# charleschen003/doudizhu-rl

Hardware: NVIDIA B200
Metric: env-steps/sec (legal moves + state encode) (higher is better)
Workload: dtype u64

## Files before the change

doudizhu-rl_b200/csrc/ddz_kernels.cu:

```cuda
#include <cuda.h>
#include <cuda_runtime.h>
#include <cstdint>
#include <cstdio>
#include <cstdlib>
#include <cstring>
#include <atomic>
#include <mutex>

#include "../../include/ddz_b200.h"
#include "ddz_device.cuh"
#include <cuda_bf16.h>
#include <math_constants.h>
#include "ddz_flat.cuh"
#include "ddz_search.cuh"

namespace ddz {

#ifndef DDZ_THREADS
#define DDZ_THREADS 64
#endif
constexpr int kThreads = DDZ_THREADS;
constexpr int kWarpsPerCta = kThreads / 32;
constexpr int kEnvs = 128;
constexpr int kWin = 320;
constexpr int kMinCtasPerSm = 28 / kWarpsPerCta;
#ifdef DDZ_PLAIN_STORES
#define DDZ_STORE(p, v) (*(p) = (v))
#else
#define DDZ_STORE(p, v) __stcs((p), (v))
#endif
#ifndef DDZ_HEAVY
#define DDZ_HEAVY 32
#endif
#ifndef DDZ_ROW_UNROLL
#define DDZ_ROW_UNROLL 4
#endif
#ifndef DDZ_LOOKBACK
#define DDZ_LOOKBACK 4
#endif
#ifndef DDZ_TILE_ENVS
#define DDZ_TILE_ENVS 32
#endif
constexpr int kTile = DDZ_TILE_ENVS;
constexpr int kRowUnroll = DDZ_ROW_UNROLL;
constexpr int kHeavy = DDZ_HEAVY;
#ifndef DDZ_PHASE_ORDER
#define DDZ_PHASE_ORDER 0
#endif
DDZ_DEV bool kFaceSecond(int t) { return DDZ_PHASE_ORDER == 0 ? (t & 1) != 0 : DDZ_PHASE_ORDER == 2; }
constexpr int kLookBack = DDZ_LOOKBACK;

enum Mode { kStepOnly = 0, kObserve = 1, kStepObserve = 2 };

#ifdef DDZ_PROB_FORM_B
constexpr int kProbForm = 1, kLutEntries = 16;
constexpr uint64_t kProbMark = 0x0008888888888888ull;
#else
constexpr int kProbForm = 0, kLutEntries = 8;
constexpr uint64_t kProbMark = 0ull;
#endif
DDZ_DEV float4 lut_entry(int i) {
    const int c = i & 7;
    return (i & 8) ? make_float4(c > 3 ? 1.f : 0.f, c > 2 ? 1.f : 0.f, c > 1 ? 1.f : 0.f, c > 0 ? 1.f : 0.f)
                   : make_float4(c > 0 ? 1.f : 0.f, c > 1 ? 1.f : 0.f, c > 2 ? 1.f : 0.f, c > 3 ? 1.f : 0.f);
}

struct WsHeader { unsigned int ticket, finished, epoch, auto_step; };
struct Workspace { WsHeader* h; unsigned long long* tile; };
static inline int ntiles(int B) { return (B + kTile - 1) / kTile; }
static inline int nblocks(int B) { return (B + kEnvs - 1) / kEnvs; }
static inline Workspace ws_of(void* p) {
    Workspace w; w.h = (WsHeader*)p; w.tile = (unsigned long long*)((char*)p + 256);
    return w;
}
constexpr unsigned long long kAggregate = 1ull << 32, kInclusive = 2ull << 32;

DDZ_DEV unsigned long long ld_relaxed(const unsigned long long* p) {
    unsigned long long v;
    asm volatile("ld.relaxed.gpu.global.u64 %0, [%1];" : "=l"(v) : "l"(p) : "memory");
    return v;
}
DDZ_DEV void st_relaxed(unsigned long long* p, unsigned long long v) {
    asm volatile("st.relaxed.gpu.global.u64 [%0], %1;" ::"l"(p), "l"(v) : "memory");
}

#ifdef DDZ_TRACE
__device__ unsigned long long* g_trace = nullptr;
DDZ_DEV void trace(int tile, int slot) {
    if (g_trace && (threadIdx.x & 31) == 0) {
        unsigned long long ts; asm volatile("mov.u64 %0, %globaltimer;" : "=l"(ts));
        g_trace[(size_t)tile * 8 + slot] = ts;
    }
}
#else
DDZ_DEV void trace(int, int) {}
#endif

DDZ_DEV long long warp_sum_ll(long long v) {
#pragma unroll
    for (int o = 16; o > 0; o >>= 1) v += __shfl_xor_sync(0xFFFFFFFFu, v, o);
    return v;
}
DDZ_DEV void stat_add(int64_t* stats, int slot, long long v) {
    const int s = __reduce_add_sync(0xFFFFFFFFu, (int)v);
    if ((threadIdx.x & 31) == 0 && s != 0 && stats) atomicAdd((unsigned long long*)&stats[slot], (unsigned long long)(long long)s);
}
DDZ_DEV void step_stats(int64_t* stats, unsigned int sf, const int32_t* rewards, int extra_err) {
    const int over = (sf >> 2) & 1, winner = (sf >> 3) & 3;
    stat_add(stats, 4, sf & 1);
    stat_add(stats, 9, (sf >> 1) & 1);
    stat_add(stats, 0, over);
    stat_add(stats, 1, over && winner == 1);
    stat_add(stats, 2, over && winner == 2);
    stat_add(stats, 3, over && winner == 0);
    stat_add(stats, 5, over ? (winner == 1 ? rewards[1] : -rewards[1]) : 0);
    stat_add(stats, 6, over ? (winner == 1 ? -(rewards[0] + rewards[2]) : rewards[0] + rewards[2]) : 0);
    stat_add(stats, 7, (int)((sf >> 5) & 3) + extra_err);
}


DDZ_DEV long long tile_lookback(const Workspace& ws, int t, unsigned long long epoch_tag, int total, int lane, int64_t* stats,
                                bool& timed_out) {
    constexpr unsigned FULL = 0xFFFFFFFFu;
    long long base = 0;
    timed_out = false;
    if (t <= 0) return 0;
    int p = t - 1;
    unsigned int spins = 0;
    bool finished = false;
    while (!finished) {
        unsigned long long w[kLookBack];
#pragma unroll
        for (int j = 0; j < kLookBack; j++) {
            const int idx = p - 32 * j - lane;
            w[j] = idx >= 0 ? ld_relaxed(&ws.tile[idx]) : (epoch_tag | kInclusive);
        }
#pragma unroll
        for (int j = 0; j < kLookBack; j++) {
            if (finished) break;
            const bool ok = ((w[j] >> 34) == (epoch_tag >> 34)) && ((w[j] >> 32) & 3ull) != 0;
            if (!__all_sync(FULL, ok)) {
                __nanosleep(64);
                if (++spins > (1u << 22)) {
                    if (lane == 0 && stats) atomicAdd((unsigned long long*)&stats[7], 1ull);
                    finished = true; timed_out = true;
                }
                break;
            }
            const unsigned int incmask = __ballot_sync(FULL, ((w[j] >> 32) & 3ull) == 2ull);
            const int stop = incmask ? (__ffs(incmask) - 1) : 31;
            base += warp_sum_ll(lane <= stop ? (long long)(unsigned int)w[j] : 0ll);
            p -= 32;
            if (incmask) finished = true;
        }
    }
    if (lane == 0) st_relaxed(&ws.tile[t], epoch_tag | kInclusive | (unsigned int)(base + total));
    return base;
}

__global__ void __launch_bounds__(kEnvs) k_reset(void* state, const int8_t* __restrict__ perm,
                                                 const int8_t* __restrict__ lord_pile, int pool_games,
                                                 int only_done, int64_t* stats, int B) {
    const int b = blockIdx.x * kEnvs + threadIdx.x, lane = threadIdx.x & 31;
    const bool valid = b < B;
    StateView v = view_of(state, B);
    Env e;
    if (valid) e = load_env(v, b); else e.meta = 0;
    const bool want = valid && (!only_done || e.done());
    const unsigned int need = __ballot_sync(0xFFFFFFFFu, want);
    const unsigned int bad = warp_deal(need, e, perm, lord_pile, pool_games, B, b, lane);
    if (want) store_env(v, b, e);
    if (lane == 0 && bad && stats) atomicAdd((unsigned long long*)&stats[7], (unsigned long long)__popc(bad));
}

struct RowLane {
    int first;
    int k;
    uint32_t sh;
    bool hi;
    DDZ_DEV static RowLane make(int lane) {
        RowLane r; r.first = lane / 15; r.k = lane - 15 * r.first; r.hi = r.k >= 8; r.sh = 4u * (uint32_t)(r.k & 7);
        if (lane >= 30) { r.first = 0x3FFFFFFF; r.k = 0; }
        return r;
    }
    DDZ_DEV const float4& thermo(uint64_t packed, const float4* lut) const {
        const uint32_t w = hi ? (uint32_t)(packed >> 32) : (uint32_t)packed;
        return lut[(w >> sh) & 15u];
    }
};
struct FaceRow { uint64_t packed; float s; float pad; };

template <class RowT>
DDZ_DEV void write_rows(float4* __restrict__ gdst, int nrows, const RowLane& rl, const float4* __restrict__ lut,
                        const RowT* __restrict__ rows);
template <>
DDZ_DEV void write_rows<FaceRow>(float4* __restrict__ gdst, int nrows, const RowLane& rl, const float4* __restrict__ lut,
                                 const FaceRow* __restrict__ rows) {
    float4* dst = gdst + (rl.first & 1) * 15 + rl.k;
#pragma unroll (kRowUnroll)
    for (int r = rl.first; r < nrows; r += 2, dst += 30) {
        const float4 raw = *reinterpret_cast<const float4*>(&rows[r]);
        const uint64_t packed = ((uint64_t)__float_as_uint(raw.y) << 32) | __float_as_uint(raw.x);
        const float s = raw.z;
        float4 q = rl.thermo(packed, lut);
        q.x *= s; q.y *= s; q.z *= s; q.w *= s;
        DDZ_STORE(dst, q);
    }
}
template <>
DDZ_DEV void write_rows<uint64_t>(float4* __restrict__ gdst, int nrows, const RowLane& rl, const float4* __restrict__ lut,
                                  const uint64_t* __restrict__ rows) {
    float4* dst = gdst + (rl.first & 1) * 15 + rl.k;
#pragma unroll (kRowUnroll)
    for (int r = rl.first; r < nrows; r += 2, dst += 30) DDZ_STORE(dst, rl.thermo(rows[r], lut));
}

template <int V> struct FaceCfg;
template <> struct FaceCfg<0> { static constexpr int C = 4; };
template <> struct FaceCfg<1> { static constexpr int C = 7; };
template <> struct FaceCfg<2> { static constexpr int C = 9; };
template <> struct FaceCfg<3> { static constexpr int C = 6; };

template <int V>
DDZ_DEV void face_planes(const Env& e, uint64_t* planes , float* p ) {
    int s = e.cur(), prev = (s + 2) % 3, next = (s + 1) % 3;
    uint64_t hand = pick3(s, e.hand[0], e.hand[1], e.hand[2]);
    uint64_t taken = e.hist[0] + e.hist[1] + e.hist[2];
    int n = 0;
    planes[n++] = hand;
    planes[n++] = taken;
    if (V == 1 || V == 2) {
        planes[n++] = pick3(prev, e.hist[0], e.hist[1], e.hist[2]);
        planes[n++] = pick3(s, e.hist[0], e.hist[1], e.hist[2]);
        planes[n++] = pick3(next, e.hist[0], e.hist[1], e.hist[2]);
    }
    if (V == 2 || V == 3) {
        planes[n++] = pick3(prev, e.recent[0], e.recent[1], e.recent[2]);
        planes[n++] = pick3(next, e.recent[0], e.recent[1], e.recent[2]);
    }
    uint64_t unknown = (kDeckPacked - taken - hand) | kProbMark;
    planes[n++] = unknown;
    planes[n++] = unknown;
    int size1 = card_count(pick3(next, e.hand[0], e.hand[1], e.hand[2]));
    int size2 = card_count(pick3(prev, e.hand[0], e.hand[1], e.hand[2]));
    int tot = size1 + size2;
    p[0] = tot > 0 ? __fdiv_rn((float)size1, (float)tot) : 0.f;
    p[1] = tot > 0 ? __fdiv_rn((float)size2, (float)tot) : 0.f;
}

struct StepArgs {
    const int32_t* offsets; const uint64_t* actions; const void* choice; int mode;
    uint64_t seed, env0; uint32_t stepno; int32_t rewards[3];
    const int8_t* perm; const int8_t* lord_pile; int pool_games;
    int8_t* r; uint8_t* done; int8_t* cat; float* reward;
    long long prev_cap;
};
struct OutArgs {
    int32_t* offsets; uint64_t* actions_u64; float4* actions_f32; long long cap; float4* face;
    int static_tiles;
};


struct SeqWindowEmitter {
    uint64_t* out; int pos, win;
    DDZ_DEV void operator()(uint64_t mv) { if ((unsigned)pos < (unsigned)win) out[pos] = mv; pos++; }
};
struct WindowEmitter {
    uint64_t* out; int base, win;
    DDZ_DEV void operator()(int idx, uint64_t mv) { const unsigned rel = (unsigned)(base + idx); if (rel < (unsigned)win) out[rel] = mv; }
};

struct __align__(128) WarpSmem {
    FaceRow face[32 * 9];
    uint64_t moves[kWin];
    float4 lut[kLutEntries];
};

template <int V, int MODE>
__global__ void __launch_bounds__(kThreads, kMinCtasPerSm) k_env(void* state, StepArgs a, OutArgs o,
                                                  Workspace ws, int64_t* stats, int B) {
    constexpr bool STEP = (MODE == kStepOnly || MODE == kStepObserve);
    constexpr bool EMIT = (MODE != kStepOnly);
    constexpr int C = FaceCfg<(V < 0 ? 0 : V)>::C;
    constexpr unsigned FULL = 0xFFFFFFFFu;
    extern __shared__ __align__(128) unsigned char smem_raw[];
    const int lane = threadIdx.x & 31, wib = threadIdx.x >> 5;
    WarpSmem& sm = reinterpret_cast<WarpSmem*>(smem_raw)[wib];
    const RowLane rl = RowLane::make(lane);
    const int nt = (B + kTile - 1) / kTile;
    const unsigned int nwarps = gridDim.x * kWarpsPerCta;

    int t = blockIdx.x * kWarpsPerCta + wib;
    unsigned int epoch = 0, autostep = 0, stepno = a.stepno;
    if (EMIT) {
        if (lane == 0) {
            if (!o.static_tiles) t = (int)atomicAdd(&ws.h->ticket, 1u);
            epoch = ws.h->epoch; autostep = ws.h->auto_step;
        }
        if (!o.static_tiles) t = __shfl_sync(FULL, t, 0);
        if (lane < kLutEntries) sm.lut[lane] = lut_entry(lane);
        __syncwarp();
    }
    if (t < nt) {
    const int b0 = t * kTile, b = b0 + lane;
    const bool valid = lane < kTile && b < B;
    const int nenv = min(kTile, B - b0);
    trace(t, 0);

    Env e;
    e.meta = 0;
    uint64_t hand = 0, last = 0;
    Masks hm{0, 0, 0, 0};
    Rule ru{true, 0, 1, 0};
    int n = 0;
    unsigned int sf = 0;
    int prev_off = 0, prev_end = 0;
    uint64_t choice_raw = 0;
    if (valid) {
        if (STEP) {
            prev_off = a.offsets[b]; prev_end = a.offsets[b + 1];
            if (a.mode == DDZ_CHOICE_MOVE) choice_raw = ((const uint64_t*)a.choice)[b];
            else if (a.mode != DDZ_CHOICE_PHILOX) choice_raw = ((const uint32_t*)a.choice)[b];
        }
        e = load_env(view_of(state, B), b);
        if (STEP && a.perm) {
            const char* prow = reinterpret_cast<const char*>(a.perm) +
                               54 * ((size_t)((e.meta >> 8) % (uint32_t)a.pool_games) * B + b);
            asm volatile("prefetch.global.L2 [%0];" ::"l"(prow));
            asm volatile("prefetch.global.L2 [%0];" ::"l"(prow + 53));
        }
    }
    if (EMIT) {
        epoch = __shfl_sync(FULL, epoch, 0);
        autostep = __shfl_sync(FULL, autostep, 0);
        if (STEP && a.stepno == DDZ_STEPNO_AUTO) stepno = autostep;
    }
    const unsigned long long epoch_tag = (unsigned long long)(epoch & 0x3FFFFFFFu) << 34;
    if (valid) {
        if (STEP) {
            int o_r = 0, o_cat = -1;
            float rw0 = 0.f, rw1 = 0.f, rw2 = 0.f;
            if (!e.done()) {
                const int base = prev_off, full = prev_end - prev_off;
                const int cnt = a.prev_cap >= 0 ? (int)max(0ll, min((long long)full, a.prev_cap - base)) : full;
                long long idx = -1;
                if (a.mode == DDZ_CHOICE_INDEX) idx = (int32_t)(uint32_t)choice_raw;
                else if (a.mode == DDZ_CHOICE_MOD) idx = cnt > 0 ? (long long)((uint32_t)choice_raw % (uint32_t)cnt) : -1;
                else if (a.mode == DDZ_CHOICE_PHILOX) idx = cnt > 0 ? (long long)(philox(a.seed, a.env0 + (uint64_t)b, stepno) % (uint32_t)cnt) : -1;
                else {
                    const uint64_t want = choice_raw;
                    for (int i = 0; i < cnt; i++) if (a.actions[base + i] == want) { idx = i; break; }
                }
                if (idx < 0 || idx >= cnt) {
                    sf += 32u;
                    if (!(cnt == 0 && full > 0)) e.meta |= 0x20u;
                } else {
                    const uint64_t mv = a.actions[base + idx];
                    StepOut so = apply_move(e, mv, a.rewards);
                    o_r = so.r; o_cat = so.cat; rw0 = so.reward[0]; rw1 = so.reward[1]; rw2 = so.reward[2];
                    sf |= 1u | (so.pass ? 2u : 0u);
                    if (so.done) sf |= 4u | ((unsigned int)so.winner << 3);
                }
            }
            if (a.r) a.r[b] = (int8_t)o_r;
            if (a.done) a.done[b] = (uint8_t)e.done();
            if (a.cat) a.cat[b] = (int8_t)o_cat;
            if (a.reward) { a.reward[3 * (size_t)b] = rw0; a.reward[3 * (size_t)b + 1] = rw1; a.reward[3 * (size_t)b + 2] = rw2; }
        }
    }
    {
        if (STEP) {
            if (a.perm) {
                const unsigned int need = __ballot_sync(FULL, valid && e.done());
                sf += ((warp_deal(need, e, a.perm, a.lord_pile, a.pool_games, B, b, lane) >> lane) & 1u) << 5;
            }
            if (valid) store_env(view_of(state, B), b, e);
        }
        if (valid && EMIT && !e.done()) {
            hand = hand_to_move(e); last = trick_of(e);
            hm = masks_of(hand); ru = rule_of(last); n = count_legal(hm, ru, last != 0);
        }
    }
    if (STEP && !EMIT) step_stats(stats, sf, a.rewards, 0);
    if (EMIT) {
    int inc = n;
#pragma unroll
    for (int d = 1; d < 32; d <<= 1) { int u = __shfl_up_sync(FULL, inc, d); if (lane >= d) inc += u; }
    const int local = inc - n;
    const int total = __shfl_sync(FULL, inc, 31);
    if (lane == 0) st_relaxed(&ws.tile[t], epoch_tag | (t == 0 ? kInclusive : kAggregate) | (unsigned int)total);

    if (V >= 0 && o.face && valid) {
        uint64_t pl[C]; float p[2];
        face_planes<(V < 0 ? 0 : V)>(e, pl, p);
#pragma unroll
        for (int c = 0; c < C; c++) {
            FaceRow fr; fr.packed = pl[c]; fr.s = (c >= C - 2) ? p[c - (C - 2)] : 1.f; fr.pad = 0.f;
            *reinterpret_cast<float4*>(&sm.face[lane * C + c]) = *reinterpret_cast<const float4*>(&fr);
        }
    }
    __syncwarp();
    trace(t, 1);

    int disagree = 0;
#pragma unroll 1
    for (int ph = 0; ph < 2; ph++) {
    if ((ph == 0) != kFaceSecond(t)) {
        trace(t, 2);
        if (V >= 0 && o.face) write_rows<FaceRow>(o.face + (size_t)b0 * C * 15, nenv * C, rl, sm.lut, sm.face);
        trace(t, 3);
    } else {
        trace(t, 4);
        long long base = 0, lim = 0;
        int w0 = 0;
        uint64_t* const wbuf = (V < 0) ? reinterpret_cast<uint64_t*>(sm.face) : sm.moves;
        const int win = (V < 0) ? (int)(sizeof(sm.face) / 8) + kWin : kWin;
#pragma unroll 1
        do {
            const bool inwin = n > 0 && local < w0 + win && local + n > w0;
            if (inwin && n <= kHeavy) {
                SeqWindowEmitter em{wbuf, local - w0, win};
                enumerate_legal(hm, ru, last != 0, em);
                disagree |= (em.pos != local - w0 + n);
            }
            unsigned int heavy = __ballot_sync(FULL, inwin && n > kHeavy);
            while (heavy) {
                const int src = __ffs(heavy) - 1; heavy &= heavy - 1;
                Masks sm_; Rule sr;
                sm_.g1 = __shfl_sync(FULL, hm.g1, src); sm_.g2 = __shfl_sync(FULL, hm.g2, src);
                sm_.g3 = __shfl_sync(FULL, hm.g3, src); sm_.g4 = __shfl_sync(FULL, hm.g4, src);
                const int rpack = __shfl_sync(FULL, (int)ru.lead | (ru.cat << 1) | (ru.len << 8) | (ru.val << 16) | ((last != 0) << 24), src);
                sr.lead = rpack & 1; sr.cat = (rpack >> 1) & 127; sr.len = (rpack >> 8) & 255; sr.val = (rpack >> 16) & 255;
                const int loc = __shfl_sync(FULL, local, src), nn = __shfl_sync(FULL, n, src);
                WindowEmitter em{wbuf, loc - w0, win};
                const int got = enumerate_legal_warp(sm_, sr, (rpack >> 24) & 1, lane, em);
                disagree |= (got != nn);
            }
            __syncwarp();
            if (w0 == 0) trace(t, 7);

            if (w0 == 0) {
                bool timed_out;
                base = tile_lookback(ws, t, epoch_tag, total, lane, stats, timed_out);
                if (valid) o.offsets[b] = (int32_t)(base + local);
                if (t == nt - 1 && lane == 0) {
                    o.offsets[B] = (int32_t)(base + total);
                    if (stats) {
                        atomicAdd((unsigned long long*)&stats[8], (unsigned long long)(base + total));
                        if (base + total > o.cap) atomicAdd((unsigned long long*)&stats[7], 1ull);
                    }
                }
                lim = o.cap - base; if (lim > total) lim = total; if (lim < 0 || timed_out) lim = 0;
                trace(t, 5);
            }

            const int keep = (int)max(0ll, min((long long)min(win, total - w0), lim - w0));
            for (int i = lane; i < keep; i += 32) o.actions_u64[base + w0 + i] = wbuf[i];
            if (o.actions_f32) write_rows<uint64_t>(o.actions_f32 + (size_t)(base + w0) * 15, keep, rl, sm.lut, wbuf);
            __syncwarp();
            w0 += win;
        } while (w0 < total);
        trace(t, 6);
    }
    }
    step_stats(stats, STEP ? sf : 0u, a.rewards, disagree);
    }
    }
    if (EMIT && lane == 0) {
        const unsigned int fin = atomicAdd(&ws.h->finished, 1u);
        if (fin == nwarps - 1) {
            ws.h->ticket = 0; ws.h->finished = 0; ws.h->epoch = epoch + 1;
            if (STEP) ws.h->auto_step = (a.stepno == DDZ_STEPNO_AUTO ? autostep : a.stepno) + 1;
            __threadfence();
        }
    }
}

#ifndef DDZ_FLAT_WARPS
#define DDZ_FLAT_WARPS 4
#endif
#ifndef DDZ_FLAT_ARENA
#define DDZ_FLAT_ARENA 512
#endif
#ifndef DDZ_FLAT_COUNT_WALK
#define DDZ_FLAT_COUNT_WALK 0
#endif
#ifndef DDZ_FLAT_MIN_CTAS
#define DDZ_FLAT_MIN_CTAS 7
#endif
#ifndef DDZ_FLAT_PAIR
#define DDZ_FLAT_PAIR 0
#endif
constexpr int kFlatWarps = DDZ_FLAT_WARPS;
constexpr int kFlatArena = DDZ_FLAT_ARENA;
__device__ const flat::SubsetTable g_subsets = flat::SubsetTable();

struct __align__(16) FlatWarpSmem {
    flat::Desc arena[kFlatArena + 2];
    uint8_t lists[32 * flat::kListsPerHand * flat::kListStride];
};

__global__ void __launch_bounds__(kFlatWarps * 32, DDZ_FLAT_MIN_CTAS) k_legal_flat(const uint64_t* __restrict__ hands,
                                                                  const uint64_t* __restrict__ lasts, OutArgs o,
                                                                  Workspace ws, int64_t* stats, int B) {
    constexpr unsigned FULL = 0xFFFFFFFFu;
    __shared__ __align__(16) uint16_t s_table[(flat::kTableSize + 7) / 8 * 8];
    __shared__ FlatWarpSmem s_warp[kFlatWarps];
    const int lane = threadIdx.x & 31, wib = threadIdx.x >> 5;
    FlatWarpSmem& sm = s_warp[wib];
    for (int i = threadIdx.x; i < flat::kTableSize; i += kFlatWarps * 32) s_table[i] = g_subsets.v[i];
    const int nt = (B + 31) / 32;
    const unsigned int nwarps = gridDim.x * kFlatWarps;
    int t = blockIdx.x * kFlatWarps + wib;
    unsigned int epoch = 0;
    if (lane == 0) {
        if (!o.static_tiles) t = (int)atomicAdd(&ws.h->ticket, 1u);
        epoch = ws.h->epoch;
    }
    if (!o.static_tiles) t = __shfl_sync(FULL, t, 0);
    __syncthreads();
    if (t < nt) {
        const int b = t * 32 + lane;
        const bool valid = b < B;
        uint64_t hand = 0, last = 0;
        if (valid) { hand = hands[b]; last = lasts[b]; }
        epoch = __shfl_sync(FULL, epoch, 0);
        const unsigned long long epoch_tag = (unsigned long long)(epoch & 0x3FFFFFFFu) << 34;
        const Masks hm = masks_of(hand);
        const Rule ru = rule_of(last);
#if DDZ_FLAT_COUNT_WALK
        flat::CountSink cs;
        if (valid) flat::walk_groups(hm, ru, last != 0, 4 * lane, cs);
        const int n = cs.n, ng = cs.ng;
#else
        const int n = valid ? count_legal(hm, ru, last != 0) : 0;
        const int ng = valid ? flat::count_groups(hm, ru, last != 0) : 0;
#endif
        int inc = n, dinc = ng;
#pragma unroll
        for (int d = 1; d < 32; d <<= 1) {
            const int u = __shfl_up_sync(FULL, inc, d), v = __shfl_up_sync(FULL, dinc, d);
            if (lane >= d) { inc += u; dinc += v; }
        }
        const int local = inc - n, total = __shfl_sync(FULL, inc, 31);
        const int dloc = dinc - ng, dtotal = __shfl_sync(FULL, dinc, 31);
        if (lane == 0) st_relaxed(&ws.tile[t], epoch_tag | (t == 0 ? kInclusive : kAggregate) | (unsigned int)total);
        if (valid) flat::write_lists(hm, 4 * lane, sm.lists);

        long long base = 0, lim = 0;
        int disagree = 0, h0 = 0;
        bool first = true;
#pragma unroll 1
        while (h0 < 32) {
            const int D0 = __shfl_sync(FULL, dloc, h0);
            const unsigned int fits = __ballot_sync(FULL, lane >= h0 && dloc + ng - D0 <= kFlatArena);
            const int h1 = h0 + __popc(fits);
            const int m0 = __shfl_sync(FULL, local, h0);
            const int m1s = __shfl_sync(FULL, local, h1 & 31), d1s = __shfl_sync(FULL, dloc, h1 & 31);
            const int m1 = h1 < 32 ? m1s : total, nd = (h1 < 32 ? d1s : dtotal) - D0;
            if (h1 == h0) { disagree = 1; break; }
            if (valid && lane >= h0 && lane < h1) {
                flat::WriteSink wsk{sm.arena, dloc - D0, kFlatArena, (uint32_t)local};
                flat::walk_groups(hm, ru, last != 0, 4 * lane, wsk);
                disagree |= (wsk.d != dloc - D0 + ng) | (wsk.start != (uint32_t)(local + n));
            }
            if (lane == 0) { flat::Desc e; e.start = (uint32_t)m1; e.prm = 0; sm.arena[nd] = e; }
            __syncwarp();
            if (first) {
                first = false;
                bool timed_out;
                base = tile_lookback(ws, t, epoch_tag, total, lane, stats, timed_out);
                if (valid) o.offsets[b] = (int32_t)(base + local);
                if (t == nt - 1 && lane == 0) {
                    o.offsets[B] = (int32_t)(base + total);
                    if (stats) {
                        atomicAdd((unsigned long long*)&stats[8], (unsigned long long)(base + total));
                        if (base + total > o.cap) atomicAdd((unsigned long long*)&stats[7], 1ull);
                    }
                }
                lim = o.cap - base; if (lim > total) lim = total; if (lim < 0 || timed_out) lim = 0;
            }
            const int mEnd = (int)min((long long)m1, lim);
            int gcur = 0;
#pragma unroll 1
            for (int w0 = m0 - (int)((base + m0) & 1); w0 < mEnd; w0 += 64) {
                uint32_t blo = 0, bhi = 0;
                for (int gq = gcur + 1;; gq += 32) {
                    const int idx = gq + lane;
                    const uint32_t rel = idx <= nd ? sm.arena[idx].start - (uint32_t)w0 : 64u;
                    blo |= rel < 32u ? 1u << rel : 0u;
                    bhi |= (rel >= 32u && rel < 64u) ? 1u << (rel - 32u) : 0u;
                    if (!__shfl_sync(FULL, (int)(rel < 64u), 31)) break;
                }
                blo = __reduce_or_sync(FULL, blo); bhi = __reduce_or_sync(FULL, bhi);
                const int x = 2 * lane;
                const uint32_t mlo = x < 31 ? (2u << x) - 1u : 0xFFFFFFFFu, mhi = x < 32 ? 0u : (2u << (x - 32)) - 1u;
                const int g0 = gcur + __popc(blo & mlo) + __popc(bhi & mhi);
                const int g1 = g0 + (int)(((x + 1 < 32) ? (blo >> (x + 1)) : (bhi >> (x - 31))) & 1u);
                const int i0 = w0 + x;
                const bool v0 = i0 >= m0 && i0 < mEnd, v1 = i0 + 1 < mEnd;
                if (v0 || v1) {
                    uint64_t mv0, mv1;
                    const flat::Desc d0 = sm.arena[g0], d1 = sm.arena[g1];
                    const int c0 = (int)(sm.arena[g0 + 1].start - d0.start), c1 = (int)(sm.arena[g1 + 1].start - d1.start);
#if DDZ_FLAT_PAIR
                    flat::decode2(d0.prm, i0 - (int)d0.start, c0, v0, d1.prm, i0 + 1 - (int)d1.start, c1, v1, s_table, sm.lists, mv0, mv1);
#else
                    mv0 = v0 ? flat::decode(d0.prm, i0 - (int)d0.start, c0, s_table, sm.lists) : 0ull;
                    mv1 = v1 ? flat::decode(d1.prm, i0 + 1 - (int)d1.start, c1, s_table, sm.lists) : 0ull;
#endif
                    uint64_t* dst = o.actions_u64 + (base + i0);
                    if (v0 && v1) *reinterpret_cast<ulonglong2*>(dst) = make_ulonglong2(mv0, mv1);
                    else if (v0) dst[0] = mv0;
                    else dst[1] = mv1;
                }
                gcur += __popc(blo) + __popc(bhi);
            }
            __syncwarp();
            h0 = h1;
// ... 447 lines not shown
        }
        return;
    }
    const int me = e.cur();
    const uint64_t env = a.env0 + (uint64_t)b;
    const int32_t zero_rewards[3] = {0, 0, 0};
    uint32_t j = 0;
    int nn = 1;
    uct_init(T, 0, e.hand, e.recent, me, -1, 0ull, -1, -1, a.prune, lane);
    __syncwarp();
    for (int it = 0; it < a.budget; it++) {
        int x = 0;
        while (T[x].winner < 0) {
            const UctNode& X = T[x];
            const int remaining = X.remaining;
            if (remaining > 0) {
                const int i = (int)(philox(a.seed, env, 0x80000000u + j++) % (uint32_t)remaining);
                const uint32_t w = lane < 16 ? X.untried[lane] : 0u;
                const int pc = __popc(w);
                int incl = pc;
#pragma unroll
                for (int o = 1; o < 32; o <<= 1) { const int v = __shfl_up_sync(FULL, incl, o); if (lane >= o) incl += v; }
                const bool mine = i >= incl - pc && i < incl;
                const int wl = __ffs(__ballot_sync(FULL, mine)) - 1;
                const int bit = mine ? (int)__fns(w, 0, i - (incl - pc) + 1) : 0;
                const int entry = __shfl_sync(FULL, wl * 32 + bit, wl);
                const int cur = X.cur;
                uint64_t hand[3] = {X.hand[0], X.hand[1], X.hand[2]}, recent[3] = {X.recent[0], X.recent[1], X.recent[2]};
                const uint64_t h = hand[cur], last = uct_trick(recent, cur);
                const Masks m = masks_of(h);
                const Rule ru = rule_of(last);
                const int n = count_legal(m, ru, last != 0);
                uint64_t mv;
                int index;
                if (a.prune && n > search::kPruneAbove) {
                    int nfull;
                    warp_mcts_list(h, last, s_moves[wib], s_keys[wib], s_list[wib], lane, nfull);
                    __syncwarp();
                    mv = s_list[wib][entry];
                    int idx = DDZ_MAX_LEGAL;
                    for (int k = lane; k < nfull; k += 32) if (s_moves[wib][k] == mv) idx = min(idx, k);
                    index = __reduce_min_sync(FULL, idx);
                    __syncwarp();
                } else {
                    mv = select_legal(m, ru, last != 0, entry);
                    index = entry;
                }
                __syncwarp();
                if (lane == wl) T[x].untried[lane] = w & ~(1u << bit);
                if (lane == 0) {
                    T[x].remaining = (int16_t)(remaining - 1);
                    if (T[x].first_child < 0) T[x].first_child = nn;
                    T[x].last_child = nn;
                    T[x].nchild += 1;
                }
                hand[cur] -= mv;
                recent[cur] = mv;
                const int winner = (mv != 0 && hand[cur] == 0) ? cur : -1;
                uct_init(T, nn, hand, recent, (cur + 1) % 3, winner, mv, x, index, a.prune, lane);
                __syncwarp();
                x = nn++;
                break;
            }
            x = uct_best_child(T, x, X.cur == me, false, a.c, a.ln[X.visits], a.seed, env, j, lane);
        }
        int reward;
        const UctNode& L = T[x];
        if (L.winner >= 0) {
            reward = ((L.winner == 1) == (me == 1)) ? a.width : 0;
        }
#ifndef DDZ_UCT_LANE_PLAYOUT
        else if (a.prune && a.width == 1) {
            Env pe;
            for (int q = 0; q < 3; q++) { pe.hand[q] = L.hand[q]; pe.hist[q] = 0; pe.recent[q] = L.recent[q]; }
            pe.meta = (uint32_t)L.cur;
            const uint64_t stream = (a.env0 + (uint64_t)b) * (uint64_t)a.budget + (uint64_t)it;
            const int winner = uct_warp_playout(pe, a.seed, stream, s_moves[wib], s_keys[wib], s_list[wib], lane);
            reward = (winner >= 0 && ((winner == 1) == (me == 1))) ? 1 : 0;
        }
#endif
        else {
            int won = 0;
            for (int w = lane; w < a.width; w += 32) {
                Env pe;
                for (int q = 0; q < 3; q++) { pe.hand[q] = L.hand[q]; pe.hist[q] = 0; pe.recent[q] = L.recent[q]; }
                pe.meta = (uint32_t)L.cur;
                int steps = 0, passes = 0, over = 0, winner = 0;
                const uint64_t stream = ((a.env0 + (uint64_t)b) * (uint64_t)a.budget + (uint64_t)it) * (uint64_t)a.width + (uint64_t)w;
                if (a.prune) playout_env<true>(pe, kUctPlayoutSteps, a.seed, stream, 0, zero_rewards, steps, passes, over, winner);
                else playout_env<false>(pe, kUctPlayoutSteps, a.seed, stream, 0, zero_rewards, steps, passes, over, winner);
                won += (over && ((winner == 1) == (me == 1))) ? 1 : 0;
            }
            reward = __reduce_add_sync(FULL, won);
        }
        __syncwarp();
        if (lane == 0)
            for (int y = x; y >= 0; y = T[y].parent) { T[y].visits += a.width; T[y].wins += reward; }
        __syncwarp();
    }
    const int best = uct_best_child(T, 0, true, true, 0.0, 0.0, a.seed, env, j, lane);
    const int nroot = T[0].nchild;
    if (a.root_n) {
        for (int k = lane; k < min(nroot, a.root_stride); k += 32) {
            const size_t o = (size_t)b * (size_t)a.root_stride + (size_t)k;
            a.root_moves[o] = T[1 + k].move; a.root_visits[o] = T[1 + k].visits; a.root_wins[o] = T[1 + k].wins;
        }
    }
    if (lane == 0) {
        a.choice[b] = T[best].index;
        if (a.move) a.move[b] = T[best].move;
        if (a.root_n) a.root_n[b] = nroot;
        *nnodes = nn;
    }
}

__global__ void __launch_bounds__(256) k_select_actions(const float* __restrict__ q, const int32_t* __restrict__ offsets,
                                                        float epsilon, uint64_t seed, uint64_t env0, uint32_t stepno,
                                                        int32_t* __restrict__ choice, int B) {
    const int b = blockIdx.x * blockDim.x + threadIdx.x;
    if (b >= B) return;
    const int lo = offsets[b], n = offsets[b + 1] - lo;
    int best = -1;
    if (n > 0) {
        bool explore = false;
        if (epsilon > 0.f) {
            const uint32_t u = philox(seed ^ 0x9E3779B97F4A7C15ull, env0 + (uint64_t)b, stepno);
            explore = (float)(u >> 8) * (1.0f / 16777216.0f) < epsilon;
            if (explore) best = (int)(philox(seed ^ 0xD1B54A32D192ED03ull, env0 + (uint64_t)b, stepno) % (uint32_t)n);
        }
        if (!explore) {
            float bv = q[lo]; best = 0;
            for (int i = 1; i < n; i++) { const float v = q[lo + i]; if (v > bv || (v != v && bv == bv)) { bv = v; best = i; } }
        }
    }
    choice[b] = best;
}

}

using namespace ddz;

static thread_local char g_err[256] = "";
static std::atomic<int> g_tile_order{DDZ_TILES_AUTO};
static int cuda_fail(cudaError_t e, const char* what) {
    snprintf(g_err, sizeof g_err, "%s: %s", what, cudaGetErrorString(e));
    return DDZ_E_CUDA;
}
#define DDZ_LAUNCH_CHECK(what)                                         \
    do {                                                               \
        cudaError_t e_ = cudaGetLastError();                           \
        if (e_ != cudaSuccess) return cuda_fail(e_, what);             \
    } while (0)

template <int V, int MODE>
static int launch_env(void* state, const StepArgs& a, const OutArgs& o, void* workspace, int64_t* stats, int B, cudaStream_t st) {
    const size_t smem = (MODE == kStepOnly) ? 0 : kWarpsPerCta * sizeof(WarpSmem);
    Workspace ws = workspace ? ws_of(workspace) : Workspace{nullptr, nullptr};
    const int grid = (ntiles(B) + kWarpsPerCta - 1) / kWarpsPerCta;
    static std::atomic<int> resident_of[64];
    static std::once_flag once;
    std::call_once(once, [] { for (auto& r : resident_of) r.store(-1); });
    int dev = 0;
    if (cudaGetDevice(&dev) != cudaSuccess) return cuda_fail(cudaGetLastError(), "cudaGetDevice");
    int resident = dev < 64 ? resident_of[dev].load(std::memory_order_relaxed) : -1;
    if (resident < 0) {
        int per_sm = 0, sms = 0;
        if (cudaDeviceGetAttribute(&sms, cudaDevAttrMultiProcessorCount, dev) != cudaSuccess ||
            cudaOccupancyMaxActiveBlocksPerMultiprocessor(&per_sm, k_env<V, MODE>, kThreads, smem) != cudaSuccess)
            return cuda_fail(cudaGetLastError(), "occupancy query");
        resident = per_sm * sms;
        if (dev < 64) resident_of[dev].store(resident, std::memory_order_relaxed);
    }
    OutArgs oo = o;
    oo.static_tiles = (g_tile_order.load(std::memory_order_relaxed) == DDZ_TILES_AUTO && grid <= resident) ? 1 : 0;
    k_env<V, MODE><<<grid, kThreads, smem, st>>>(state, a, oo, ws, stats, B);
    DDZ_LAUNCH_CHECK("k_env");
    return 0;
}
template <int V>
static int launch_q_features(const void* state, const int32_t* offsets, const uint64_t* actions, const uint8_t* env_mask,
                             const int32_t* dst_offsets, int env_begin, int env_count, long long row_base, const float* T,
                             const float* rank_bias, const float* L, const float* line_bias, int W, void* out, int out_bf16,
                             int B, cudaStream_t st) {
    const size_t smem = (size_t)5 * kQThreads * sizeof(float4);
    const float4* T4 = reinterpret_cast<const float4*>(T);
    const float4* rb4 = reinterpret_cast<const float4*>(rank_bias);
#define DDZ_Q_LAUNCH(BF, WC_) k_q_features<V, BF, WC_><<<env_count, kQThreads, smem, st>>>(                        \
        state, offsets, actions, env_mask, dst_offsets, env_begin, row_base, T4, rb4, L, line_bias, W, out, B)
    if (W == 256) { if (out_bf16) DDZ_Q_LAUNCH(true, 256); else DDZ_Q_LAUNCH(false, 256); }
    else          { if (out_bf16) DDZ_Q_LAUNCH(true, 0); else DDZ_Q_LAUNCH(false, 0); }
#undef DDZ_Q_LAUNCH
    DDZ_LAUNCH_CHECK("k_q_features");
    return 0;
}
template <int MODE>
static int launch_env_v(int variant, bool want_face, void* state, const StepArgs& a, const OutArgs& o, void* workspace,
                        int64_t* stats, int B, cudaStream_t st) {
    if (!want_face) return launch_env<-1, MODE>(state, a, o, workspace, stats, B, st);
    switch (variant) {
        case 0: return launch_env<0, MODE>(state, a, o, workspace, stats, B, st);
        case 1: return launch_env<1, MODE>(state, a, o, workspace, stats, B, st);
        case 2: return launch_env<2, MODE>(state, a, o, workspace, stats, B, st);
        case 3: return launch_env<3, MODE>(state, a, o, workspace, stats, B, st);
    }
    return DDZ_E_ARG;
}

namespace {
struct DriverApi {
    CUresult (*getGranularity)(size_t*, const CUmemAllocationProp*, CUmemAllocationGranularity_flags);
    CUresult (*create)(CUmemGenericAllocationHandle*, size_t, const CUmemAllocationProp*, unsigned long long);
    CUresult (*release)(CUmemGenericAllocationHandle);
    CUresult (*reserve)(CUdeviceptr*, size_t, size_t, CUdeviceptr, unsigned long long);
    CUresult (*addressFree)(CUdeviceptr, size_t);
    CUresult (*map)(CUdeviceptr, size_t, size_t, CUmemGenericAllocationHandle, unsigned long long);
    CUresult (*unmap)(CUdeviceptr, size_t);
    CUresult (*setAccess)(CUdeviceptr, size_t, const CUmemAccessDesc*, size_t);
    bool ok;
};
template <class Fn>
bool driver_fn(const char* name, Fn& fn) {
    void* p = nullptr;
    cudaDriverEntryPointQueryResult st;
    if (cudaGetDriverEntryPoint(name, &p, cudaEnableDefault, &st) != cudaSuccess || st != cudaDriverEntryPointSuccess || !p) {
        cudaGetLastError();
        return false;
    }
    fn = reinterpret_cast<Fn>(p);
    return true;
}
const DriverApi& driver_api() {
    static DriverApi d = [] {
        DriverApi a{};
        a.ok = driver_fn("cuMemGetAllocationGranularity", a.getGranularity) && driver_fn("cuMemCreate", a.create) &&
               driver_fn("cuMemRelease", a.release) && driver_fn("cuMemAddressReserve", a.reserve) &&
               driver_fn("cuMemAddressFree", a.addressFree) && driver_fn("cuMemMap", a.map) &&
               driver_fn("cuMemUnmap", a.unmap) && driver_fn("cuMemSetAccess", a.setAccess);
        return a;
    }();
    return d;
}
}

extern "C" {

#ifdef DDZ_TRACE
int ddz_debug_set_trace(unsigned long long* buf) {
    return cudaMemcpyToSymbol(g_trace, &buf, sizeof buf) == cudaSuccess ? 0 : DDZ_E_CUDA;
}
#endif
int ddz_abi_version(void) { return DDZ_ABI_VERSION; }
int ddz_prob_form(void) { return kProbForm; }
int ddz_set_tile_order(int mode) {
    if (mode != DDZ_TILES_AUTO && mode != DDZ_TILES_TICKET) return DDZ_E_ARG;
    return g_tile_order.exchange(mode);
}
int ddz_face_channels(int variant) {
    static const int C[4] = {4, 7, 9, 6};
    return (variant < 0 || variant > 3) ? DDZ_E_ARG : C[variant];
}
size_t ddz_state_bytes(int B) { return B <= 0 ? 0 : (size_t)B * (9 * 8 + 4); }
size_t ddz_workspace_bytes(int B) { return B <= 0 ? 0 : 256 + (size_t)ntiles(B) * 8; }
const char* ddz_last_error(void) { return g_err; }

int ddz_reset(void* state, const int8_t* perm, const int8_t* lord_pile, int pool_games, int only_done,
              int64_t* stats, int B, void* stream) {
    if (!state || !perm || B <= 0 || pool_games < 1) return DDZ_E_ARG;
    k_reset<<<nblocks(B), kEnvs, 0, (cudaStream_t)stream>>>(state, perm, lord_pile, pool_games, only_done, stats, B);
    DDZ_LAUNCH_CHECK("k_reset");
    return 0;
}

int ddz_observe(const void* state, void* workspace, int variant, int32_t* offsets, uint64_t* actions_u64,
                float* actions_f32, int64_t cap, float* face, int64_t* stats, int B, void* stream) {
    if (!state || !workspace || !offsets || !actions_u64 || B <= 0 || cap < 0) return DDZ_E_ARG;
    if (face && ddz_face_channels(variant) < 0) return DDZ_E_ARG;
    StepArgs a; memset(&a, 0, sizeof a);
    OutArgs o{offsets, actions_u64, (float4*)actions_f32, cap, (float4*)face, 0};
    return launch_env_v<kObserve>(variant, face != nullptr, const_cast<void*>(state), a, o, workspace, stats, B,
                                  (cudaStream_t)stream);
}

int ddz_legal_count(const void* state, int32_t* counts, int B, void* stream) {
    if (!state || !counts || B <= 0) return DDZ_E_ARG;
    k_legal_count<<<(B + 255) / 256, 256, 0, (cudaStream_t)stream>>>(state, counts, B);
    DDZ_LAUNCH_CHECK("k_legal_count");
    return 0;
}

int ddz_legal_emit(const void* state, void* workspace, int32_t* offsets, uint64_t* actions_u64, int64_t cap,
                   int64_t* stats, int B, void* stream) {
    return ddz_observe(state, workspace, 0, offsets, actions_u64, nullptr, cap, nullptr, stats, B, stream);
}

static int fill_step_args(StepArgs& a, const int32_t* offsets, const uint64_t* actions, const void* choice, int mode,
                          uint64_t seed, uint64_t env0, uint32_t stepno, const int32_t rewards[3], int8_t* r,
                          uint8_t* done, int8_t* cat, float* reward) {
    static const int32_t defR[3] = {50, 100, 50};
    if (!offsets || !actions || mode < 0 || mode > 3) return DDZ_E_ARG;
    if (mode != DDZ_CHOICE_PHILOX && !choice) return DDZ_E_ARG;
    memset(&a, 0, sizeof a);
    a.offsets = offsets; a.actions = actions; a.choice = choice; a.mode = mode;
    a.seed = seed; a.env0 = env0; a.stepno = stepno;
    for (int i = 0; i < 3; i++) a.rewards[i] = rewards ? rewards[i] : defR[i];
    a.r = r; a.done = done; a.cat = cat; a.reward = reward;
    a.pool_games = 1;
    a.prev_cap = -1;
    return 0;
}

int ddz_step(void* state, const int32_t* offsets, const uint64_t* actions_u64, const void* choice,
             int choice_mode, uint64_t seed, uint64_t env0, uint32_t stepno, const int32_t rewards[3],
             int8_t* r, uint8_t* done, int8_t* cat, float* reward, int64_t* stats, int B, void* stream) {
    if (!state || B <= 0) return DDZ_E_ARG;
    StepArgs a;
    int rc = fill_step_args(a, offsets, actions_u64, choice, choice_mode, seed, env0, stepno, rewards, r, done, cat, reward);
    if (rc) return rc;
    OutArgs o{nullptr, nullptr, nullptr, 0, nullptr, 0};
    return launch_env<-1, kStepOnly>(state, a, o, nullptr, stats, B, (cudaStream_t)stream);
}

int ddz_rollout_step(void* state, void* workspace, int variant,
                     const int32_t* prev_offsets, const uint64_t* prev_actions_u64,
                     const void* choice, int choice_mode, uint64_t seed, uint64_t env0, uint32_t stepno,
                     const int32_t rewards[3], const int8_t* perm, const int8_t* lord_pile, int pool_games,
                     int8_t* r, uint8_t* done, int8_t* cat, float* reward,
                     int32_t* out_offsets, uint64_t* out_actions_u64, float* out_actions_f32, int64_t cap,
                     float* face, int64_t* stats, int B, void* stream) {
    if (!state || !workspace || !out_offsets || !out_actions_u64 || B <= 0 || cap < 0) return DDZ_E_ARG;
    if (out_offsets == prev_offsets || (cap > 0 && out_actions_u64 == prev_actions_u64)) return DDZ_E_ARG;
// ... 474 lines not shown
```

Baseline: 1.609 billion.

## Add warp-specialized face-writer warp fed by rule warps via named barriers

Introduces a CTA shape with several rule warps (legal-move enumeration and action emission) plus one dedicated face-writer warp. Each rule warp stages its face planes in shared memory and signals the writer through a named barrier, so face-row stores overlap with move enumeration instead of running as a serialized phase in every warp. This path is used when the grid fits in resident CTAs, otherwise the old shape runs. It adds named-barrier synchronization and changes CTA size and occupancy, and the single writer warp can become a bottleneck if face output dominates.

```diff
diff --git a/doudizhu-rl_b200/csrc/ddz_kernels.cu b/doudizhu-rl_b200/csrc/ddz_kernels.cu
--- a/doudizhu-rl_b200/csrc/ddz_kernels.cu
+++ b/doudizhu-rl_b200/csrc/ddz_kernels.cu
@@ -23,7 +23,10 @@
 constexpr int kWarpsPerCta = kThreads / 32;
 constexpr int kEnvs = 128;
 constexpr int kWin = 320;
-constexpr int kMinCtasPerSm = 28 / kWarpsPerCta;
+#ifndef DDZ_WARPS_PER_SM
+#define DDZ_WARPS_PER_SM 28
+#endif
+constexpr int kWarpsPerSm = DDZ_WARPS_PER_SM;
 #ifdef DDZ_PLAIN_STORES
 #define DDZ_STORE(p, v) (*(p) = (v))
 #else
@@ -49,6 +52,13 @@
 #endif
 DDZ_DEV bool kFaceSecond(int t) { return DDZ_PHASE_ORDER == 0 ? (t & 1) != 0 : DDZ_PHASE_ORDER == 2; }
 constexpr int kLookBack = DDZ_LOOKBACK;
+#ifndef DDZ_FACE_WRITER
+#define DDZ_FACE_WRITER 1
+#endif
+#ifndef DDZ_RULE_WARPS
+#define DDZ_RULE_WARPS 3
+#endif
+static_assert(DDZ_RULE_WARPS >= 0 && DDZ_RULE_WARPS <= 15, "rule warp j uses named barrier j + 1: ids 1..15");
 
 enum Mode { kStepOnly = 0, kObserve = 1, kStepObserve = 2 };
 
@@ -275,22 +285,64 @@
     uint64_t moves[kWin];
     float4 lut[kLutEntries];
 };
-
-template <int V, int MODE>
-__global__ void __launch_bounds__(kThreads, kMinCtasPerSm) k_env(void* state, StepArgs a, OutArgs o,
-                                                  Workspace ws, int64_t* stats, int B) {
+struct FaceWarpSmem {
+    float4 lut[kLutEntries];
+    int tile[DDZ_RULE_WARPS > 0 ? DDZ_RULE_WARPS : 1];
+};
+
+template <int V, int MODE, bool ROLES> struct EnvCta {
+    static constexpr bool kRoles = ROLES && DDZ_FACE_WRITER && DDZ_RULE_WARPS > 0 && V >= 0 && MODE != kStepOnly;
+    static constexpr int kTiles = kRoles ? DDZ_RULE_WARPS : kWarpsPerCta;
+    static constexpr int kWarps = kRoles ? DDZ_RULE_WARPS + 1 : kWarpsPerCta;
+    static constexpr int kThreads = 32 * kWarps;
+    static constexpr int kMinCtas = kWarpsPerSm / kWarps;
+    static constexpr size_t kSmem = MODE == kStepOnly ? 0 : kTiles * sizeof(WarpSmem) + (kRoles ? sizeof(FaceWarpSmem) : 0);
+    static_assert(kMinCtas >= 1, "DDZ_WARPS_PER_SM must hold at least one CTA");
+};
+DDZ_DEV void bar_arrive(int id, int nthreads) { asm volatile("bar.arrive %0, %1;" ::"r"(id), "r"(nthreads) : "memory"); }
+DDZ_DEV void bar_sync(int id, int nthreads) { asm volatile("bar.sync %0, %1;" ::"r"(id), "r"(nthreads) : "memory"); }
+
+template <int C, int R>
+DDZ_DEV void face_warp(const WarpSmem* sm, FaceWarpSmem& fw, float4* face, int B, int lane) {
+    const RowLane rl = RowLane::make(lane);
+    const int nt = (B + kTile - 1) / kTile;
+    if (lane < kLutEntries) fw.lut[lane] = lut_entry(lane);
+    __syncwarp();
+#pragma unroll 1
+    for (int j = 0; j < R; j++) {
+        bar_sync(j + 1, 64);
+        const int t = fw.tile[j];
+        if (t < nt && face) {
+            const int b0 = t * kTile;
+            trace(t, 2);
+            write_rows<FaceRow>(face + (size_t)b0 * C * 15, min(kTile, B - b0) * C, rl, fw.lut, sm[j].face);
+            trace(t, 3);
+        }
+    }
+}
+
+template <int V, int MODE, bool WANT_ROLES>
+__global__ void __launch_bounds__(EnvCta<V, MODE, WANT_ROLES>::kThreads, EnvCta<V, MODE, WANT_ROLES>::kMinCtas)
+k_env(void* state, StepArgs a, OutArgs o, Workspace ws, int64_t* stats, int B) {
     constexpr bool STEP = (MODE == kStepOnly || MODE == kStepObserve);
     constexpr bool EMIT = (MODE != kStepOnly);
+    constexpr bool ROLES = EnvCta<V, MODE, WANT_ROLES>::kRoles;
+    constexpr int TILES = EnvCta<V, MODE, WANT_ROLES>::kTiles;
     constexpr int C = FaceCfg<(V < 0 ? 0 : V)>::C;
     constexpr unsigned FULL = 0xFFFFFFFFu;
     extern __shared__ __align__(128) unsigned char smem_raw[];
     const int lane = threadIdx.x & 31, wib = threadIdx.x >> 5;
+    FaceWarpSmem& fw = *reinterpret_cast<FaceWarpSmem*>(smem_raw + TILES * sizeof(WarpSmem));
+    if (ROLES && wib == TILES) {
+        face_warp<C, TILES>(reinterpret_cast<const WarpSmem*>(smem_raw), fw, o.face, B, lane);
+        return;
+    }
     WarpSmem& sm = reinterpret_cast<WarpSmem*>(smem_raw)[wib];
     const RowLane rl = RowLane::make(lane);
     const int nt = (B + kTile - 1) / kTile;
-    const unsigned int nwarps = gridDim.x * kWarpsPerCta;
-
-    int t = blockIdx.x * kWarpsPerCta + wib;
+    const unsigned int nwarps = gridDim.x * TILES;
+
+    int t = blockIdx.x * TILES + wib;
     unsigned int epoch = 0, autostep = 0, stepno = a.stepno;
     if (EMIT) {
         if (lane == 0) {
@@ -298,6 +350,7 @@
             epoch = ws.h->epoch; autostep = ws.h->auto_step;
         }
         if (!o.static_tiles) t = __shfl_sync(FULL, t, 0);
+        if (ROLES && lane == 0) fw.tile[wib] = t;
         if (lane < kLutEntries) sm.lut[lane] = lut_entry(lane);
         __syncwarp();
     }
@@ -401,11 +454,12 @@
     }
     __syncwarp();
     trace(t, 1);
+    if (ROLES) bar_arrive(wib + 1, 64);
 
     int disagree = 0;
 #pragma unroll 1
-    for (int ph = 0; ph < 2; ph++) {
-    if ((ph == 0) != kFaceSecond(t)) {
+    for (int ph = ROLES ? 1 : 0; ph < 2; ph++) {
+    if (!ROLES && (ph == 0) != kFaceSecond(t)) {
         trace(t, 2);
         if (V >= 0 && o.face) write_rows<FaceRow>(o.face + (size_t)b0 * C * 15, nenv * C, rl, sm.lut, sm.face);
         trace(t, 3);
@@ -465,6 +519,8 @@
     }
     step_stats(stats, STEP ? sf : 0u, a.rewards, disagree);
     }
+    } else if (ROLES) {
+        bar_arrive(wib + 1, 64);
     }
     if (EMIT && lane == 0) {
         const unsigned int fin = atomicAdd(&ws.h->finished, 1u);
@@ -1218,30 +1274,47 @@
         if (e_ != cudaSuccess) return cuda_fail(e_, what);             \
     } while (0)
 
-template <int V, int MODE>
-static int launch_env(void* state, const StepArgs& a, const OutArgs& o, void* workspace, int64_t* stats, int B, cudaStream_t st) {
-    const size_t smem = (MODE == kStepOnly) ? 0 : kWarpsPerCta * sizeof(WarpSmem);
-    Workspace ws = workspace ? ws_of(workspace) : Workspace{nullptr, nullptr};
-    const int grid = (ntiles(B) + kWarpsPerCta - 1) / kWarpsPerCta;
+template <int V, int MODE, bool ROLES>
+static int resident_ctas(int& resident) {
+    using Cta = EnvCta<V, MODE, ROLES>;
     static std::atomic<int> resident_of[64];
     static std::once_flag once;
     std::call_once(once, [] { for (auto& r : resident_of) r.store(-1); });
     int dev = 0;
     if (cudaGetDevice(&dev) != cudaSuccess) return cuda_fail(cudaGetLastError(), "cudaGetDevice");
-    int resident = dev < 64 ? resident_of[dev].load(std::memory_order_relaxed) : -1;
+    resident = dev < 64 ? resident_of[dev].load(std::memory_order_relaxed) : -1;
     if (resident < 0) {
         int per_sm = 0, sms = 0;
         if (cudaDeviceGetAttribute(&sms, cudaDevAttrMultiProcessorCount, dev) != cudaSuccess ||
-            cudaOccupancyMaxActiveBlocksPerMultiprocessor(&per_sm, k_env<V, MODE>, kThreads, smem) != cudaSuccess)
+            cudaOccupancyMaxActiveBlocksPerMultiprocessor(&per_sm, k_env<V, MODE, ROLES>, Cta::kThreads, Cta::kSmem) != cudaSuccess)
             return cuda_fail(cudaGetLastError(), "occupancy query");
         resident = per_sm * sms;
         if (dev < 64) resident_of[dev].store(resident, std::memory_order_relaxed);
     }
+    return 0;
+}
+template <int V, int MODE, bool ROLES>
+static int launch_env_shape(void* state, const StepArgs& a, const OutArgs& o, void* workspace, int64_t* stats, int B,
+                            int grid, int resident, cudaStream_t st) {
+    using Cta = EnvCta<V, MODE, ROLES>;
+    Workspace ws = workspace ? ws_of(workspace) : Workspace{nullptr, nullptr};
     OutArgs oo = o;
     oo.static_tiles = (g_tile_order.load(std::memory_order_relaxed) == DDZ_TILES_AUTO && grid <= resident) ? 1 : 0;
-    k_env<V, MODE><<<grid, kThreads, smem, st>>>(state, a, oo, ws, stats, B);
+    k_env<V, MODE, ROLES><<<grid, Cta::kThreads, Cta::kSmem, st>>>(state, a, oo, ws, stats, B);
     DDZ_LAUNCH_CHECK("k_env");
     return 0;
+}
+template <int V, int MODE>
+static int launch_env(void* state, const StepArgs& a, const OutArgs& o, void* workspace, int64_t* stats, int B, cudaStream_t st) {
+    int resident = 0, rc = 0;
+    if constexpr (EnvCta<V, MODE, true>::kRoles) {
+        const int grid = (ntiles(B) + EnvCta<V, MODE, true>::kTiles - 1) / EnvCta<V, MODE, true>::kTiles;
+        if ((rc = resident_ctas<V, MODE, true>(resident)) != 0) return rc;
+        if (grid <= resident) return launch_env_shape<V, MODE, true>(state, a, o, workspace, stats, B, grid, resident, st);
+    }
+    const int grid = (ntiles(B) + kWarpsPerCta - 1) / kWarpsPerCta;
+    if ((rc = resident_ctas<V, MODE, false>(resident)) != 0) return rc;
+    return launch_env_shape<V, MODE, false>(state, a, o, workspace, stats, B, grid, resident, st);
 }
 template <int V>
 static int launch_q_features(const void* state, const int32_t* offsets, const uint64_t* actions, const uint8_t* env_mask,
```

Result: faster. 1.739 billion, median of 6 (+8.1%).
